# quanpn90/avsr

Hardware: AMD Instinct MI355X
Metric: AV-frames/sec/GPU (fwd+bwd) on 15s clips; WER parity on LRS2 test (higher is better)
Workload: dtype bf16

## Files before the change

### avsr_amd/csrc/gemm.hip

```cpp
#include "gemm_core.h"
#include "gemm_glds.h"
#include "gemm_pp.h"
#include <algorithm>
#include <cstring>

using namespace gemmcore;

namespace {

struct DenseArgs {
  int M, N, K, splits, kchunk;
  uint32_t a_bytes, b_bytes;
  int64_t sSplit;
  const void* A; int64_t lda, sA;
  const void* B; int64_t ldb, sB;
  int64_t sC, sR;
  Epi e;
  unsigned long long* stamp;
  unsigned* cnt;
  float* fC; int64_t fldc;
  float falpha, fbeta;
  const float* ln_c1; float ln_eps;
  float* lnst;
  float* kvk; float* kvv; const int* kvpos; int kvrows;
};

template <typename T, typename OutT, int WM, int WN, bool AK, bool BK>
__global__ __launch_bounds__(NT) void dense_kernel(DenseArgs a) {
  extern __shared__ __attribute__((aligned(16))) char smem[];
  using TL = Tile<T, WM, WN, AK, BK>;
  const int z = blockIdx.z, bz = z / a.splits, sp = z % a.splits;
  const int m0 = blockIdx.y * TL::BM, n0 = blockIdx.x * TL::BN;
  using LA = typename std::conditional<AK, LdDenseK<T, TL::BM>, LdDenseR<T, TL::BM>>::type;
  using LB = typename std::conditional<BK, LdDenseK<T, TL::BN>, LdDenseR<T, TL::BN>>::type;
  LA la; la.p = (const T*)a.A + (int64_t)bz * a.sA; la.ld = a.lda; la.rext = a.M; la.K = a.K;
  LB lb; lb.p = (const T*)a.B + (int64_t)bz * a.sB; lb.ld = a.ldb; lb.rext = a.N; lb.K = a.K;
  const int kbeg = sp * a.kchunk, kend = min(a.K, kbeg + a.kchunk);
  f32x16 acc[2][2];
  mainloop<T, WM, WN>(la, lb, m0, n0, kbeg, kend, acc, smem);
  Epi e = a.e;
  e.C = (OutT*)e.C + (int64_t)bz * a.sC + sp * a.sSplit;
  if (e.res) e.res = (const T*)e.res + (int64_t)bz * a.sR;
  if (e.preact) e.preact = (T*)e.preact + (int64_t)bz * a.sC;
  if (e.gate) e.gate = (const T*)e.gate + (int64_t)bz * a.sC;
  e.drop_base = (uint64_t)bz * (uint64_t)a.M * (uint64_t)a.N;
  epilogue<T, OutT, WM, WN>(e, m0, n0, acc, smem);
}

template <typename OutT, bool AK, bool BK, class CF>
__global__ __launch_bounds__(CF::NTH, CF::MINB) void dense_glds_kernel(DenseArgs a, int tiles_m, int tiles_n) {
  extern __shared__ __attribute__((aligned(16))) char smem[];
  if (a.stamp != nullptr && threadIdx.x == 0) atomicMin(a.stamp, (unsigned long long)__builtin_amdgcn_s_memrealtime());
  const int id = gemmg::xcd_remap(blockIdx.x, gridDim.x);
  int tm, tn, z;
  gemmg::tile_of(id, tiles_m, tiles_n, tm, tn, z);
  const int bz = z / a.splits, sp = z % a.splits;
  const int m0 = tm * CF::BM, n0 = tn * CF::BN;
  const int kbeg = sp * a.kchunk, kend = min(a.K, kbeg + a.kchunk);
  const int lane = threadIdx.x & 63, wave = __builtin_amdgcn_readfirstlane(threadIdx.x >> 6);
  f32x4 acc[CF::TM][CF::TN];
  const int nk = (kend - kbeg + gemmg::GBK - 1) / gemmg::GBK;
  if (a.a_bytes) {
    using LA = typename std::conditional<AK, gemmg::BDenseK<CF::BM, CF::NW>, gemmg::BDenseR<CF::BM, CF::NW>>::type;
    using LB = typename std::conditional<BK, gemmg::BDenseK<CF::BN, CF::NW>, gemmg::BDenseR<CF::BN, CF::NW>>::type;
    LA la; la.init((const bf16*)a.A + (int64_t)bz * a.sA, a.a_bytes, a.lda, m0, a.M, kend, wave, lane);
    LB lb; lb.init((const bf16*)a.B + (int64_t)bz * a.sB, a.b_bytes, a.ldb, n0, a.N, kend, wave, lane);
    gemmg::mainloop_glds<CF>(la, lb, kbeg, nk, acc, smem);
  } else {
    using LA = typename std::conditional<AK, gemmg::GDenseK<CF::BM, CF::NW>, gemmg::GDenseR<CF::BM, CF::NW>>::type;
    using LB = typename std::conditional<BK, gemmg::GDenseK<CF::BN, CF::NW>, gemmg::GDenseR<CF::BN, CF::NW>>::type;
    LA la; la.init((const bf16*)a.A + (int64_t)bz * a.sA, a.lda, m0, a.M, kend, wave, lane);
    LB lb; lb.init((const bf16*)a.B + (int64_t)bz * a.sB, a.ldb, n0, a.N, kend, wave, lane);
    gemmg::mainloop_glds<CF>(la, lb, kbeg, nk, acc, smem);
  }
  Epi e = a.e;
  e.C = (OutT*)e.C + (int64_t)bz * a.sC + sp * a.sSplit;
  if (e.res) e.res = (const bf16*)e.res + (int64_t)bz * a.sR;
  if (e.preact) e.preact = (bf16*)e.preact + (int64_t)bz * a.sC;
  if (e.gate) e.gate = (const bf16*)e.gate + (int64_t)bz * a.sC;
  e.drop_base = (uint64_t)bz * (uint64_t)a.M * (uint64_t)a.N;
  gemmg::epilogue_g<bf16, OutT, CF>(e, m0, n0, acc, smem);
  if (a.stamp != nullptr) {
    __syncthreads();
    if (threadIdx.x == 0) atomicMax(a.stamp + 1, (unsigned long long)__builtin_amdgcn_s_memrealtime());
  }
}

template <class CF, bool FR>
__device__ __forceinline__ void wgrad_dual_body(const DenseArgs& a, int tiles_m, int tiles_n, int id, char* smem) {
  static_assert(CF::BM * (CF::BN + 4) * 4 <= 2 * CF::S * CF::STAGE, "reduction tile exceeds the two rings");
  if (a.stamp != nullptr && threadIdx.x == 0) atomicMin(a.stamp, (unsigned long long)__builtin_amdgcn_s_memrealtime());
  int tm, tn, sp;
  if (a.cnt) {
    int z;
    gemmg::tile_of(id / a.splits, tiles_m, tiles_n, tm, tn, z);
    sp = id % a.splits;
  } else {
    gemmg::tile_of(id, tiles_m, tiles_n, tm, tn, sp);
  }
  const int m0 = tm * CF::BM, n0 = tn * CF::BN;
  const int kbeg = sp * a.kchunk, kend = min(a.K, kbeg + a.kchunk);
  const int lane = threadIdx.x & 63;
  const int wv = __builtin_amdgcn_readfirstlane(threadIdx.x >> 6);
  const int grp = wv >> 2, wave = wv & 3;
  const int ntile = (kend - kbeg + gemmg::GBK - 1) / gemmg::GBK;
  const int nk = (ntile + 1) >> 1;
  const int gbeg = kbeg + grp * nk * gemmg::GBK, gend = min(kend, gbeg + nk * gemmg::GBK);
  f32x4 acc[CF::TM][CF::TN];
  char* ring = smem + grp * (CF::S * CF::STAGE);
  if (a.a_bytes) {
    gemmg::BDenseR<CF::BM, CF::NW> la; la.init((const bf16*)a.A, a.a_bytes, a.lda, m0, a.M, gend, wave, lane);
    gemmg::BDenseR<CF::BN, CF::NW> lb; lb.init((const bf16*)a.B, a.b_bytes, a.ldb, n0, a.N, gend, wave, lane);
    gemmg::mainloop_glds<CF>(la, lb, gbeg, nk, acc, ring, wave);
  } else {
    gemmg::GDenseR<CF::BM, CF::NW> la; la.init((const bf16*)a.A, a.lda, m0, a.M, gend, wave, lane);
    gemmg::GDenseR<CF::BN, CF::NW> lb; lb.init((const bf16*)a.B, a.ldb, n0, a.N, gend, wave, lane);
    gemmg::mainloop_glds<CF>(la, lb, gbeg, nk, acc, ring, wave);
  }
  constexpr int LDR = CF::BN + 4;
  float* st = (float*)smem;
  const int wm = wave / CF::WN, wn = wave % CF::WN;
#pragma unroll
  for (int i = 0; i < CF::TM; ++i)
#pragma unroll
    for (int j = 0; j < CF::TN; ++j)
#pragma unroll
      for (int r = 0; r < 4; ++r) {
        const int row = wm * 32 * CF::FM + 16 * i + 4 * (lane >> 4) + r, col = wn * 32 * CF::FN + 16 * j + (lane & 15);
        if (grp == 0) st[row * LDR + col] = acc[i][j][r];
      }
  __syncthreads();
#pragma unroll
  for (int i = 0; i < CF::TM; ++i)
#pragma unroll
    for (int j = 0; j < CF::TN; ++j)
#pragma unroll
      for (int r = 0; r < 4; ++r) {
        const int row = wm * 32 * CF::FM + 16 * i + 4 * (lane >> 4) + r, col = wn * 32 * CF::FN + 16 * j + (lane & 15);
        if (grp == 1) st[row * LDR + col] += acc[i][j][r];
      }
  __syncthreads();
  const bool slab = a.sSplit != 0;
  constexpr int Q = CF::BN / 4;
  if constexpr (FR) {
    float* W = (float*)a.e.C;
    const int64_t ldw = a.e.ldc;
    const __amdgpu_buffer_rsrc_t rs = gemmg::make_rsrc(W, (uint32_t)((int64_t)a.splits * a.sSplit * 4));
    for (int c = threadIdx.x; c < CF::BM * Q; c += 2 * CF::NTH) {
      const int lr = c / Q, lc = (c % Q) * 4, row = m0 + lr, col = n0 + lc;
      if (row >= a.M || col >= a.N) continue;
      const f32x4 v = *(const f32x4*)(st + lr * LDR + lc);
      const uint32_t off = (uint32_t)((sp * a.sSplit + (int64_t)row * ldw + col) * 4);
      __builtin_amdgcn_raw_buffer_store_b128(__builtin_bit_cast(v4i32, v), rs, off, 0, 16 );
    }
    asm volatile("s_waitcnt vmcnt(0)" ::: "memory");
    __shared__ int last;
    __syncthreads();
    const int tile = tm * tiles_n + tn;
    if (threadIdx.x == 0)
      last = __hip_atomic_fetch_add(&a.cnt[tile], 1u, __ATOMIC_RELAXED, __HIP_MEMORY_SCOPE_AGENT) == (unsigned)a.splits - 1;
    __syncthreads();
    if (last) {
      constexpr int NI = CF::BM * Q / (2 * CF::NTH), SMAX = 4;
      static_assert(NI * 2 * CF::NTH == CF::BM * Q, "tile vectors per thread");
// ... 54 lines not shown
    }
    return;
  }
  float* C = slab ? (float*)a.e.C + sp * a.sSplit : (float*)a.e.C;
  const int64_t ldc = a.e.ldc;
  const float alpha = slab ? 1.f : a.e.alpha, beta = slab ? 0.f : a.e.beta;
  for (int c = threadIdx.x; c < CF::BM * Q; c += 2 * CF::NTH) {
    const int lr = c / Q, lc = (c % Q) * 4, row = m0 + lr, col = n0 + lc;
    if (row >= a.M || col >= a.N) continue;
    const f32x4 v = *(const f32x4*)(st + lr * LDR + lc);
    float* o = C + (int64_t)row * ldc + col;
    if (col + 4 <= a.N) {
      f32x4 y = v * alpha;
      if (beta != 0.f) y += *(const f32x4*)o * beta;
      *(f32x4*)o = y;
    } else {
      for (int q = 0; q < a.N - col; ++q) o[q] = beta != 0.f ? alpha * v[q] + beta * o[q] : alpha * v[q];
    }
  }
  if (a.stamp != nullptr) {
    __syncthreads();
    if (threadIdx.x == 0) atomicMax(a.stamp + 1, (unsigned long long)__builtin_amdgcn_s_memrealtime());
  }
}

template <class CF, bool FR = false>
__global__ __launch_bounds__(2 * CF::NTH, 1) void wgrad_dual_kernel(DenseArgs a, int tiles_m, int tiles_n) {
  extern __shared__ __attribute__((aligned(16))) char smem[];
  wgrad_dual_body<CF, FR>(a, tiles_m, tiles_n, gemmg::xcd_remap(blockIdx.x, gridDim.x), smem);
}

constexpr int WG_MAX = 4;
struct WgGroup {
  DenseArgs a[WG_MAX];
  int tm[WG_MAX], tn[WG_MAX], start[WG_MAX + 1];
};
template <class CF>
__global__ __launch_bounds__(2 * CF::NTH, 1) void wgrad_group_kernel(WgGroup g) {
  extern __shared__ __attribute__((aligned(16))) char smem[];
  const int id = gemmg::xcd_remap(blockIdx.x, gridDim.x);
  int q = 0;
#pragma unroll
  for (int i = 1; i < WG_MAX; ++i) q += id >= g.start[i];
  q = __builtin_amdgcn_readfirstlane(q);
  wgrad_dual_body<CF, false>(g.a[q], g.tm[q], g.tn[q], id - g.start[q], smem);
}

template <typename OutT, bool AK, bool BK>
__global__ __launch_bounds__(gemmpp::NTH, 1) void dense_pp_kernel(DenseArgs a, int tiles_m, int tiles_n) {
  extern __shared__ __attribute__((aligned(16))) char smem[];
  const int id = gemmg::xcd_remap(blockIdx.x, gridDim.x);
  int tm, tn, z;
  gemmg::tile_of(id, tiles_m, tiles_n, tm, tn, z);
  const int bz = z / a.splits, sp = z % a.splits;
  const int m0 = tm * gemmpp::BM, n0 = tn * gemmpp::BN;
  const int kbeg = sp * a.kchunk, kend = min(a.K, kbeg + a.kchunk);
  const int lane = threadIdx.x & 63, wave = __builtin_amdgcn_readfirstlane(threadIdx.x >> 6);
  using LA = typename std::conditional<AK, gemmpp::HalfK<64>, gemmpp::HalfR<64>>::type;
  using LB = typename std::conditional<BK, gemmpp::HalfK<32>, gemmpp::HalfR<32>>::type;
  LA la; la.init((const bf16*)a.A + (int64_t)bz * a.sA, a.lda, m0, a.M, kend, wave, lane);
  LB lb; lb.init((const bf16*)a.B + (int64_t)bz * a.sB, a.ldb, n0, a.N, kend, wave, lane);
  f32x4 acc[8][4];
  gemmpp::mainloop_pp(la, lb, kbeg, (kend - kbeg + gemmg::GBK - 1) / gemmg::GBK, acc, smem);
  Epi e = a.e;
  e.C = (OutT*)e.C + (int64_t)bz * a.sC + sp * a.sSplit;
  if (e.res) e.res = (const bf16*)e.res + (int64_t)bz * a.sR;
  if (e.preact) e.preact = (bf16*)e.preact + (int64_t)bz * a.sC;
  if (e.gate) e.gate = (const bf16*)e.gate + (int64_t)bz * a.sC;
  e.drop_base = (uint64_t)bz * (uint64_t)a.M * (uint64_t)a.N;
  gemmg::epilogue_g<bf16, OutT, gemmpp::CF>(e, m0, n0, acc, smem);
}

template <typename OutT, bool AK, bool BK>
int launch_pp(const DenseArgs& a, int batch, hipStream_t st) {
  const int tm = (a.M + 255) / 256, tn = (a.N + 255) / 256;
  const long nwg = (long)tm * tn * batch * a.splits;
  if (nwg > 0x7fffffffL) return AVSR_E_SHAPE;
  hipLaunchKernelGGL((dense_pp_kernel<OutT, AK, BK>), dim3((unsigned)nwg), dim3(gemmpp::NTH), gemmpp::LDS_BYTES, st, a,
                     tm, tn);
  AVSR_CHECK_LAUNCH();
  return 0;
}

template <typename OutT, bool AK, bool BK, class CF>
int launch_glds(const DenseArgs& a, int batch, hipStream_t st) {
  const int tm = (a.M + CF::BM - 1) / CF::BM, tn = (a.N + CF::BN - 1) / CF::BN;
  const long nwg = (long)tm * tn * batch * a.splits;
  if (nwg > 0x7fffffffL) return AVSR_E_SHAPE;
  hipLaunchKernelGGL((dense_glds_kernel<OutT, AK, BK, CF>), dim3((unsigned)nwg), dim3(CF::NTH), CF::LDS_BYTES, st, a,
                     tm, tn);
  AVSR_CHECK_LAUNCH();
  return 0;
}

using Cfg128 = gemmg::GCfg<2, 2, 2, 2, 2>;
using Cfg256 = gemmg::GCfg<2, 4, 4, 2, 2>;
using Cfg256x128 = gemmg::GCfg<4, 2, 2, 2, 3>;
using Cfg128x256 = gemmg::GCfg<2, 4, 2, 2, 3>;
using Cfg128s3 = gemmg::GCfg<2, 2, 2, 2, 3>;
using Cfg128s4 = gemmg::GCfg<2, 2, 2, 2, 4>;
using Cfg128w8s3 = gemmg::GCfg<2, 4, 2, 1, 3>;
using Cfg128w8s4 = gemmg::GCfg<2, 4, 2, 1, 4>;
using Cfg96 = gemmg::GCfg<3, 2, 1, 2, 2>;
using Cfg128x64 = gemmg::GCfg<4, 1, 1, 2, 2>;
using Cfg192 = gemmg::GCfg<2, 2, 3, 2, 2>;
using Cfg192x256 = gemmg::GCfg<2, 4, 3, 2, 2>;
using Cfg192s3 = gemmg::GCfg<2, 2, 3, 2, 3>;
using Cfg192w8 = gemmg::GCfg<2, 4, 3, 1, 2>;
using Cfg192w8s3 = gemmg::GCfg<2, 4, 3, 1, 3>;
using Cfg64 = gemmg::GCfg<2, 2, 1, 1, 2>;
using Cfg64s4 = gemmg::GCfg<2, 2, 1, 1, 4>;
using Cfg192w8s4 = gemmg::GCfg<2, 4, 3, 1, 4>;

#ifndef AVSR_AB_FWD2
#define AVSR_AB_FWD2 11
#endif
#ifndef AVSR_AB_ROUND1
#define AVSR_AB_ROUND1 15
#endif
int tile_cfg(const avsr_gemm_params* p, int splits) {
  const int forced = (int)avsr_opt(AVSR_OPT_GEMM_TILE) - 1;
  if (forced >= 0) return forced;
  if (p->a_kmajor) {
    const long tiles_z = (long)p->batch * splits;
    const long t128 = (long)((p->M + 127) / 128) * ((p->N + 127) / 128) * tiles_z;
    const long t192 = (long)((p->M + 191) / 192) * ((p->N + 127) / 128) * tiles_z;
    const long n128 = (t128 + 255) / 256, n192 = (t192 + 255) / 256;
    if (n192 >= 2 && 3 * n192 * 50 <= 2 * n128 * 51) return AVSR_AB_FWD2;
    if (t192 > 128 && t192 <= 256) return AVSR_AB_ROUND1;
  }
  {
    const long tiles_z = (long)p->batch * splits;
    const long t128 = (long)((p->M + 127) / 128) * ((p->N + 127) / 128) * tiles_z;
    const long t64 = (long)((p->M + 63) / 64) * ((p->N + 63) / 64) * tiles_z;
    if (t128 < 256 && t64 >= 2 * t128) return (t64 <= 256 && p->K >= 2048) ? 18 : 16;
  }
  return 0;
}

int cfg_bm(int cfg, bool ak) {
  switch (cfg) {
    case 1: return Cfg256::BM;
    case 2: return Cfg256x128::BM;
    case 3: return Cfg128x256::BM;
    case 4: return Cfg128s3::BM;
    case 5: return Cfg128s4::BM;
    case 6: return Cfg128w8s3::BM;
    case 7: return Cfg128w8s4::BM;
    case 8: return gemmpp::BM;
    case 9: return ak ? Cfg96::BM : Cfg128::BM;
    case 10: return Cfg128x64::BM;
    case 16: return Cfg64::BM;
    case 18: return Cfg64s4::BM;
    case 11: return ak ? Cfg192::BM : Cfg128::BM;
    case 12: return ak ? Cfg192x256::BM : Cfg128::BM;
    case 13: return ak ? Cfg192s3::BM : Cfg128::BM;
    case 14: return ak ? Cfg192w8::BM : Cfg128::BM;
    case 15: return ak ? Cfg192w8s3::BM : Cfg128::BM;
    case 17: return ak ? Cfg192w8s4::BM : Cfg128::BM;
    default: return Cfg128::BM;
  }
}

template <typename OutT, bool AK, bool BK>
int launch_cfg(int cfg, const DenseArgs& a, int batch, hipStream_t st) {
  switch (cfg) {
    case 1: return launch_glds<OutT, AK, BK, Cfg256>(a, batch, st);
    case 2: return launch_glds<OutT, AK, BK, Cfg256x128>(a, batch, st);
    case 3: return launch_glds<OutT, AK, BK, Cfg128x256>(a, batch, st);
    case 4: return launch_glds<OutT, AK, BK, Cfg128s3>(a, batch, st);
    case 5: return launch_glds<OutT, AK, BK, Cfg128s4>(a, batch, st);
    case 6: return launch_glds<OutT, AK, BK, Cfg128w8s3>(a, batch, st);
    case 7: return launch_glds<OutT, AK, BK, Cfg128w8s4>(a, batch, st);
    case 8: return launch_pp<OutT, AK, BK>(a, batch, st);
    case 9:
      if constexpr (AK) return launch_glds<OutT, AK, BK, Cfg96>(a, batch, st);
      else return launch_glds<OutT, AK, BK, Cfg128>(a, batch, st);
    case 10: return launch_glds<OutT, AK, BK, Cfg128x64>(a, batch, st);
    case 16: return launch_glds<OutT, AK, BK, Cfg64>(a, batch, st);
    case 18: return launch_glds<OutT, AK, BK, Cfg64s4>(a, batch, st);
    case 11:
      if constexpr (AK) return launch_glds<OutT, AK, BK, Cfg192>(a, batch, st);
      else return launch_glds<OutT, AK, BK, Cfg128>(a, batch, st);
    case 12:
      if constexpr (AK) return launch_glds<OutT, AK, BK, Cfg192x256>(a, batch, st);
      else return launch_glds<OutT, AK, BK, Cfg128>(a, batch, st);
    case 13:
      if constexpr (AK) return launch_glds<OutT, AK, BK, Cfg192s3>(a, batch, st);
      else return launch_glds<OutT, AK, BK, Cfg128>(a, batch, st);
    case 14:
      if constexpr (AK) return launch_glds<OutT, AK, BK, Cfg192w8>(a, batch, st);
      else return launch_glds<OutT, AK, BK, Cfg128>(a, batch, st);
    case 15:
      if constexpr (AK) return launch_glds<OutT, AK, BK, Cfg192w8s3>(a, batch, st);
      else return launch_glds<OutT, AK, BK, Cfg128>(a, batch, st);
    case 17:
      if constexpr (AK) return launch_glds<OutT, AK, BK, Cfg192w8s4>(a, batch, st);
      else return launch_glds<OutT, AK, BK, Cfg128>(a, batch, st);
    default: return launch_glds<OutT, AK, BK, Cfg128>(a, batch, st);
  }
}

template <typename OutT>
int glds_by_layout(const avsr_gemm_params* p, const DenseArgs& a, hipStream_t st) {
  const int cfg = tile_cfg(p, a.splits);
  if (p->a_kmajor && p->b_kmajor) return launch_cfg<OutT, true, true>(cfg, a, p->batch, st);
  if (p->a_kmajor) return launch_cfg<OutT, true, false>(cfg, a, p->batch, st);
  if (p->b_kmajor) return launch_cfg<OutT, false, true>(cfg, a, p->batch, st);
  return launch_cfg<OutT, false, false>(cfg, a, p->batch, st);
}

bool glds_ok(const avsr_gemm_params* p) {
  if (p->dtype != AVSR_BF16 || p->M < 128 || p->N < 128) return false;
  if (!p->a_kmajor && (p->M % 8)) return false;
  if (!p->b_kmajor && (p->N % 8)) return false;
  return true;
}

template <typename T, typename OutT, int WM, int WN, bool AK, bool BK>
int launch(const DenseArgs& a, int batch, hipStream_t st) {
  using TL = Tile<T, WM, WN, AK, BK>;
  dim3 grid((a.N + TL::BN - 1) / TL::BN, (a.M + TL::BM - 1) / TL::BM, batch * a.splits);
  hipLaunchKernelGGL((dense_kernel<T, OutT, WM, WN, AK, BK>), grid, dim3(NT), TL::LDS_BYTES, st, a);
  AVSR_CHECK_LAUNCH();
  return 0;
}

template <typename T, typename OutT, int WM, int WN>
int by_layout(const avsr_gemm_params* p, const DenseArgs& a, hipStream_t st) {
  if (p->a_kmajor && p->b_kmajor) return launch<T, OutT, WM, WN, true, true>(a, p->batch, st);
  if (p->a_kmajor) return launch<T, OutT, WM, WN, true, false>(a, p->batch, st);
  if (p->b_kmajor) return launch<T, OutT, WM, WN, false, true>(a, p->batch, st);
  return launch<T, OutT, WM, WN, false, false>(a, p->batch, st);
}

template <typename T, typename OutT>
int by_tile(const avsr_gemm_params* p, const DenseArgs& a, hipStream_t st) {
  if (p->N <= 64) return by_layout<T, OutT, 4, 1>(p, a, st);
  if (p->M <= 64) return by_layout<T, OutT, 1, 4>(p, a, st);
  return by_layout<T, OutT, 2, 2>(p, a, st);
}

constexpr int SK_NB = 16;

template <typename T> AVSR_DEV f32x4 ld4f(const T* p) {
  if constexpr (sizeof(T) == 2) {
    const bf16x4 v = *(const bf16x4*)p;
    return f32x4{(float)v[0], (float)v[1], (float)v[2], (float)v[3]};
  } else {
    return *(const f32x4*)p;
  }
}

template <typename T, typename OutT, int MR>
__global__ __launch_bounds__(256) void skinny_kernel(DenseArgs a, float* part, int kchunk, unsigned* cnt) {
  constexpr int SK_KC = MR <= 32 ? 256 : 128;
  constexpr int XPT = MR * SK_KC / 4 / 256;
  constexpr int WJ = SK_KC / 128;
  __shared__ __attribute__((aligned(16))) float xs[MR][SK_KC + 4];
  static_assert(4 * MR * (SK_NB + 1) <= MR * (SK_KC + 4), "reduction slab reuses the staging buffer");
  float (*red)[MR][SK_NB + 1] = (float (*)[MR][SK_NB + 1])&xs[0][0];
  const int tid = threadIdx.x, cg = tid & 7, kl = tid >> 3, lane = tid & 63, wave = tid >> 6;
  const int n0 = blockIdx.x * SK_NB, c0 = n0 + 2 * cg, c1 = c0 + 1;
  const T* A = (const T*)a.A;
  const T* B0 = (const T*)a.B + (int64_t)min(c0, a.N - 1) * a.ldb;
  const T* B1 = (const T*)a.B + (int64_t)min(c1, a.N - 1) * a.ldb;
  const bool ok0 = c0 < a.N, ok1 = c1 < a.N;
  float acc0[MR], acc1[MR];
#pragma unroll
  for (int m = 0; m < MR; ++m) acc0[m] = acc1[m] = 0.f;
  const int kbeg = part ? blockIdx.y * kchunk : 0;
  const int kend = part ? min(a.K, kbeg + kchunk) : a.K;
  f32x4 xr[XPT], w0[WJ], w1[WJ];
  auto load = [&](int k0) {
#pragma unroll
    for (int i = 0; i < XPT; ++i) {
      const int idx = tid + 256 * i, m = idx / (SK_KC / 4), q = idx - m * (SK_KC / 4), k = k0 + 4 * q;
// ... 551 lines not shown
```

### avsr_amd/csrc/gemm_core.h

```cpp
#pragma once
#include "common.h"

namespace gemmcore {

constexpr int BKE = 32, NT = 256;

template <typename T> struct V { static constexpr int VE = 16 / (int)sizeof(T); static constexpr int ROW = BKE + VE; };

AVSR_DEV void zero(v16& v) { v.w[0] = v.w[1] = v.w[2] = v.w[3] = 0u; }

struct ConvGeom {
  int nimg, hin, win, hout, wout;
  int kh, kw, sh, sw, ph, pw;
  int cin, cout;
  int64_t ldx, ldy;
  FastDiv f_hw_out, f_w_out;
  FastDiv f_hw_in, f_w_in;
  FastDiv f_kw;
  int cin_shift, cout_shift;
  int ktot_w, tap_kfw, tap_kh0, tap_kw0, tap_step;
};

template <typename T, int R> struct LdDenseK {
  static constexpr bool KMAJ = true;
// ... 251 lines not shown
  void* preact;
  const void* res; int64_t ldr;
  const void* gate;
  float drop_p; uint64_t seed; uint64_t drop_base;
  float* stats;
  int stats_tiles;
  int rm_wc, rm_hc, rm_hin, rm_win, rm_a, rm_b;
  float* colsum;
};

AVSR_DEV int epi_row(const Epi& e, int r) {
  if (e.rm_wc == 0) return r;
  const int q = r / e.rm_wc, j = r - q * e.rm_wc;
  const int n = q / e.rm_hc, i = q - n * e.rm_hc;
  return (n * e.rm_hin + 2 * i + e.rm_a) * e.rm_win + 2 * j + e.rm_b;
}

AVSR_DEV int acc_row(int wm, int i, int r, int lane) { return wm * 64 + i * 32 + (r & 3) + 8 * (r >> 2) + 4 * (lane >> 5); }
AVSR_DEV int acc_col(int wn, int j, int lane) { return wn * 64 + j * 32 + (lane & 31); }

template <typename T, typename OutT, int NE>
AVSR_DEV void epi_elems(const Epi& e, int row, int col, const float* v_in) {
  OutT* C = (OutT*)e.C;
  const T* R = (const T*)e.res;
  T* P = (T*)e.preact;
  const T* G = (const T*)e.gate;
  const int64_t off = (int64_t)row * e.ldc + col;
  if (e.atomic) {
#pragma unroll
    for (int q = 0; q < NE; ++q)
      if (col + q < e.N) atomicAdd((float*)C + off + q, e.alpha * v_in[q]);
    return;
  }
#pragma unroll
  for (int q = 0; q < NE; ++q) {
    if (col + q >= e.N) break;
    float v = e.alpha * v_in[q];
    const uint64_t didx = e.drop_base + (uint64_t)row * (uint64_t)e.N + col + q;
    if (!e.bwd) {
      if (e.bias) v += e.bias[col + q];
      if (P) P[off + q] = from_f<T>(v);
      v = act_fwd_t<T>(e.act, v);
      if (e.drop_p > 0.f) v *= drop_scale(e.drop_p, e.seed, didx);
      if (R) v += to_f(R[(int64_t)row * e.ldr + col + q]);
    } else {
      if (e.drop_p > 0.f) v *= drop_scale(e.drop_p, e.seed, didx);
      if (G) v *= act_bwd_t<T>(e.act, to_f(G[off + q]));
    }
    if (e.beta != 0.f) v += e.beta * to_f(C[off + q]);
    C[off + q] = from_f<OutT>(v);
  }
}

template <typename T, typename OutT>
AVSR_DEV bool epi_vec_ok(const Epi& e) {
  const uintptr_t a = (uintptr_t)e.C | (uintptr_t)e.preact | (uintptr_t)e.res | (uintptr_t)e.gate | (uintptr_t)e.bias;
  return !e.atomic && (a & 15u) == 0 && ((e.ldc * (int64_t)sizeof(OutT)) & 15) == 0 &&
         ((e.ldc * (int64_t)sizeof(T)) & 15) == 0 && ((e.ldr * (int64_t)sizeof(T)) & 15) == 0;
}

template <typename T> AVSR_DEV void ld8(const T* p, float (&o)[8]) {
  if constexpr (sizeof(T) == 2) {
    const bf16x8 x = *(const bf16x8*)p;
#pragma unroll
    for (int j = 0; j < 8; ++j) o[j] = (float)x[j];
  } else {
    const f32x4 x0 = *(const f32x4*)p, x1 = *(const f32x4*)(p + 4);
#pragma unroll
    for (int j = 0; j < 4; ++j) { o[j] = x0[j]; o[j + 4] = x1[j]; }
  }
}
template <typename T> AVSR_DEV void st8(T* p, const float (&o)[8]) {
  if constexpr (sizeof(T) == 2) {
    bf16x8 x;
#pragma unroll
    for (int j = 0; j < 8; ++j) x[j] = (bf16)o[j];
    *(bf16x8*)p = x;
  } else {
    *(f32x4*)p = f32x4{o[0], o[1], o[2], o[3]};
    *(f32x4*)(p + 4) = f32x4{o[4], o[5], o[6], o[7]};
  }
}

template <typename T, typename OutT>
AVSR_DEV void epi_vec8(const Epi& e, int row, int col, float (&v)[8]) {
  const int64_t off = (int64_t)row * e.ldc + col;
#pragma unroll
  for (int q = 0; q < 8; ++q) v[q] *= e.alpha;
  float t[8];
  const uint64_t d0 = e.drop_base + (uint64_t)row * (uint64_t)e.N + col;
  if (!e.bwd) {
    if (e.bias) {
      ld8(e.bias + col, t);
#pragma unroll
      for (int q = 0; q < 8; ++q) v[q] += t[q];
    }
    if (e.preact) st8((T*)e.preact + off, v);
    if (e.act) {
      if (sizeof(T) == 2 && e.act == AVSR_ACT_GELU) {
#pragma unroll
        for (int q = 0; q < 8; q += 2) {
          const f32x2 r = gelu_fast2(f32x2{v[q], v[q + 1]});
          v[q] = r.x; v[q + 1] = r.y;
        }
      } else {
#pragma unroll
        for (int q = 0; q < 8; ++q) v[q] = act_fwd_t<T>(e.act, v[q]);
      }
    }
    if (e.drop_p > 0.f) drop8(e.drop_p, e.seed, d0, v);
    if (e.res) {
      ld8((const T*)e.res + (int64_t)row * e.ldr + col, t);
#pragma unroll
      for (int q = 0; q < 8; ++q) v[q] += t[q];
    }
  } else {
    if (e.drop_p > 0.f) drop8(e.drop_p, e.seed, d0, v);
    if (e.gate) {
      ld8((const T*)e.gate + off, t);
      if (sizeof(T) == 2 && e.act == AVSR_ACT_GELU) {
#pragma unroll
        for (int q = 0; q < 8; q += 2) {
          const f32x2 r = gelu_fast_grad2(f32x2{t[q], t[q + 1]});
          v[q] *= r.x; v[q + 1] *= r.y;
        }
      } else {
#pragma unroll
        for (int q = 0; q < 8; ++q) v[q] *= act_bwd_t<T>(e.act, t[q]);
      }
    }
  }
  if (e.beta != 0.f) {
    ld8((const OutT*)e.C + off, t);
#pragma unroll
    for (int q = 0; q < 8; ++q) v[q] += e.beta * t[q];
  }
  st8((OutT*)e.C + off, v);
}

template <typename T, typename OutT, int WM, int WN>
AVSR_DEV void epilogue(const Epi& e, int m0, int n0, f32x16 (&acc)[2][2], char* smem) {
  constexpr int BM = 64 * WM, BN = 64 * WN, HR = BM / 2, LDR = BN + 4;
  const int tid = threadIdx.x, lane = tid & 63, wid = tid >> 6;
  const int wm = wid / WN, wn = wid % WN;
  float* st = (float*)smem;
  if (e.stats) {
    __syncthreads();
    float* red = st;
#pragma unroll
    for (int j = 0; j < 2; ++j) {
      float s = 0.f, c = 0.f;
#pragma unroll
      for (int i = 0; i < 2; ++i)
#pragma unroll
        for (int r = 0; r < 16; ++r) {
          const bool ok = m0 + acc_row(wm, i, r, lane) < e.M;
          s += ok ? e.alpha * acc[i][j][r] : 0.f;
          c += ok ? 1.f : 0.f;
        }
      s += __shfl_xor(s, 32, 64);
      c += __shfl_xor(c, 32, 64);
      const float mean = c > 0.f ? s / c : 0.f;
      float m2 = 0.f;
#pragma unroll
      for (int i = 0; i < 2; ++i)
#pragma unroll
        for (int r = 0; r < 16; ++r) {
          const bool ok = m0 + acc_row(wm, i, r, lane) < e.M;
          const float d = e.alpha * acc[i][j][r] - mean;
          m2 += ok ? d * d : 0.f;
        }
      m2 += __shfl_xor(m2, 32, 64);
      if (lane < 32) {
        const int lc = acc_col(wn, j, lane);
        red[(wm * BN + lc) * 3 + 0] = c;
        red[(wm * BN + lc) * 3 + 1] = mean;
        red[(wm * BN + lc) * 3 + 2] = m2;
      }
    }
    __syncthreads();
    for (int lc = tid; lc < BN; lc += NT) {
      const int col = n0 + lc;
      if (col < e.N) {
        float n = 0.f, mean = 0.f, m2 = 0.f;
        for (int w = 0; w < WM; ++w) {
          const float nb = red[(w * BN + lc) * 3 + 0], mb = red[(w * BN + lc) * 3 + 1], qb = red[(w * BN + lc) * 3 + 2];
          if (nb > 0.f) {
            const float nn = n + nb, d = mb - mean;
            mean += d * nb / nn;
            m2 += qb + d * d * n * nb / nn;
            n = nn;
          }
        }
        float* o = e.stats + ((int64_t)col * e.stats_tiles + m0 / BM) * 3;
        o[0] = n; o[1] = mean; o[2] = m2;
      }
    }
  }
#pragma unroll
  for (int half = 0; half < 2; ++half) {
    __syncthreads();
#pragma unroll
// ... 40 lines not shown
```

### avsr_amd/csrc/gemm_glds.h

```cpp
#pragma once
#include "gemm_core.h"

namespace gemmg {
using namespace gemmcore;

constexpr int GBK = 64;

static __device__ __attribute__((aligned(16))) uint4 g_zero_line[64];

typedef __attribute__((address_space(3))) void lds_void_t;
typedef const __attribute__((address_space(1))) void gbl_void_t;

AVSR_DEV void glds16(const void* src, char* lds_wave_base) {
  __builtin_amdgcn_global_load_lds((gbl_void_t*)src, (lds_void_t*)lds_wave_base, 16, 0, 0);
}

template <int CPR> AVSR_DEV int rswz(int k) {
  return CPR >= 16 ? ((k & 3) | (((k >> 3) & 1) << 2)) << 1 : (((k >> 1) & 1) | (((k >> 3) & 1) << 1)) << 1;
}

template <int R, int NW> struct GDenseK {
  static constexpr bool KMAJ = true;
  static constexpr int SLOTS = R / 8 / NW;
  const bf16* p[SLOTS];
// ... 142 lines not shown
  static constexpr int LDS_BYTES = S * STAGE > EP_BYTES ? S * STAGE : EP_BYTES;
  static constexpr int MINB = LDS_BYTES <= 53 * 1024 ? 3 : LDS_BYTES <= 80 * 1024 ? 2 : 1;
  static constexpr int TM = 2 * FM, TN = 2 * FN;
};

template <int N> AVSR_DEV void wait_vmcnt() { asm volatile("s_waitcnt vmcnt(%0)" ::"n"(N) : "memory"); }

template <class CF, bool AK, bool BK>
struct Frags {
  bf16x8 a[CF::TM], b[CF::TN];
  AVSR_DEV void load(const char* stage, int kb, int wm, int wn, int lane) {
#pragma unroll
    for (int i = 0; i < CF::TM; ++i) a[i] = gfrag<CF::BM, AK>(stage, (wm * CF::TM + i) * 16, kb, lane);
#pragma unroll
    for (int j = 0; j < CF::TN; ++j) b[j] = gfrag<CF::BN, BK>(stage + CF::SA, (wn * CF::TN + j) * 16, kb, lane);
  }
  AVSR_DEV void mma(f32x4 (&acc)[CF::TM][CF::TN]) const {
#pragma unroll
    for (int i = 0; i < CF::TM; ++i)
#pragma unroll
      for (int j = 0; j < CF::TN; ++j) acc[i][j] = mfma16(a[i], b[j], acc[i][j]);
  }
};

template <class CF>
AVSR_DEV void wait_tiles_ahead(bool full) {
  if (full) wait_vmcnt<CF::GL * (CF::S - 2)>();
  else wait_vmcnt<0>();
}

template <class CF, class LA, class LB>
AVSR_DEV void mainloop_glds(const LA& la, const LB& lb, int kbeg, int nk, f32x4 (&acc)[CF::TM][CF::TN], char* smem,
                            int wave) {
  constexpr int S = CF::S, KS = GBK / 32;
  const int lane = threadIdx.x & 63;
  const int wm = wave / CF::WN, wn = wave % CF::WN;
#pragma unroll
  for (int i = 0; i < CF::TM; ++i)
#pragma unroll
    for (int j = 0; j < CF::TN; ++j) acc[i][j] = f32x4{0.f, 0.f, 0.f, 0.f};
  if (nk <= 0) return;
#pragma unroll
  for (int p = 0; p < S; ++p)
    if (p < nk) {
      la.issue(smem + p * CF::STAGE, kbeg + p * GBK, wave);
      lb.issue(smem + p * CF::STAGE + CF::SA, kbeg + p * GBK, wave);
    }
  if (nk >= S) wait_vmcnt<CF::GL * (S - 1)>();
  else wait_vmcnt<0>();
  __builtin_amdgcn_s_barrier();
  asm volatile("" ::: "memory");
  static_assert(KS == 2, "the fragment sets alternate over two k-steps per K-tile");
  Frags<CF, LA::KMAJ, LB::KMAJ> f0, f1;
  f0.load(smem, 0, wm, wn, lane);
  int cs = 0;
  for (int kt = 0; kt < nk; ++kt) {
    const char* stage = smem + cs * CF::STAGE;
    const int ns = cs + 1 == S ? 0 : cs + 1;
    f1.load(stage, 1, wm, wn, lane);
    f0.mma(acc);
    if (kt + 1 < nk) {
      asm volatile("s_waitcnt lgkmcnt(0)" ::: "memory");
      wait_tiles_ahead<CF>(kt + S - 1 < nk);
      __builtin_amdgcn_s_barrier();
      asm volatile("" ::: "memory");
      if (kt + S < nk) {
        char* st = smem + cs * CF::STAGE;
        la.issue(st, kbeg + (kt + S) * GBK, wave);
        lb.issue(st + CF::SA, kbeg + (kt + S) * GBK, wave);
      }
      f0.load(smem + ns * CF::STAGE, 0, wm, wn, lane);
    }
    f1.mma(acc);
    cs = ns;
  }
  __syncthreads();
}

template <class CF, class LA, class LB>
AVSR_DEV void mainloop_glds(const LA& la, const LB& lb, int kbeg, int nk, f32x4 (&acc)[CF::TM][CF::TN], char* smem) {
  mainloop_glds<CF>(la, lb, kbeg, nk, acc, smem, __builtin_amdgcn_readfirstlane(threadIdx.x >> 6));
}

template <typename T, typename OutT, class CF>
AVSR_DEV void epilogue_g(const Epi& e, int m0, int n0, f32x4 (&acc)[CF::TM][CF::TN], char* smem) {
  constexpr int BN = CF::BN, LDR = BN + 4, SR = CF::WM * 32;
  const int tid = threadIdx.x, lane = tid & 63, wave = tid >> 6;
  const int wm = wave / CF::WN, wn = wave % CF::WN;
  float* st = (float*)smem;
  const bool vec = epi_vec_ok<T, OutT>(e);
  if (e.stats) {
    __syncthreads();
    float* red = st;
#pragma unroll
    for (int j = 0; j < CF::TN; ++j) {
      float s = 0.f, c = 0.f;
#pragma unroll
      for (int i = 0; i < CF::TM; ++i)
#pragma unroll
        for (int r = 0; r < 4; ++r) {
          const int row = wm * 32 * CF::FM + i * 16 + 4 * (lane >> 4) + r;
          const bool ok = m0 + row < e.M;
          s += ok ? e.alpha * acc[i][j][r] : 0.f;
          c += ok ? 1.f : 0.f;
        }
      s += __shfl_xor(s, 16, 64); s += __shfl_xor(s, 32, 64);
      c += __shfl_xor(c, 16, 64); c += __shfl_xor(c, 32, 64);
      const float mean = c > 0.f ? s / c : 0.f;
      float m2 = 0.f;
#pragma unroll
      for (int i = 0; i < CF::TM; ++i)
#pragma unroll
        for (int r = 0; r < 4; ++r) {
          const int row = wm * 32 * CF::FM + i * 16 + 4 * (lane >> 4) + r;
          const float d = e.alpha * acc[i][j][r] - mean;
          m2 += m0 + row < e.M ? d * d : 0.f;
        }
      m2 += __shfl_xor(m2, 16, 64); m2 += __shfl_xor(m2, 32, 64);
      if (lane < 16) {
        const int lc = (wn * CF::TN + j) * 16 + lane;
        red[(wm * BN + lc) * 3 + 0] = c;
        red[(wm * BN + lc) * 3 + 1] = mean;
        red[(wm * BN + lc) * 3 + 2] = m2;
      }
    }
    __syncthreads();
    for (int lc = tid; lc < BN; lc += CF::NTH) {
      const int col = n0 + lc;
      if (col < e.N) {
        float n = 0.f, mean = 0.f, m2 = 0.f;
        for (int w = 0; w < CF::WM; ++w) {
          const float nb = red[(w * BN + lc) * 3 + 0], mb = red[(w * BN + lc) * 3 + 1], qb = red[(w * BN + lc) * 3 + 2];
          if (nb > 0.f) {
            const float nn = n + nb, d = mb - mean;
            mean += d * nb / nn;
            m2 += qb + d * d * n * nb / nn;
            n = nn;
          }
        }
        float* o = e.stats + ((int64_t)col * e.stats_tiles + m0 / CF::BM) * 3;
        o[0] = n; o[1] = mean; o[2] = m2;
      }
    }
  }
  static_assert(CF::NTH % (BN / 8) == 0, "a thread's column group must be fixed");
  float cs[8];
#pragma unroll
  for (int j = 0; j < 8; ++j) cs[j] = 0.f;
#pragma unroll
  for (int i = 0; i < CF::FM; ++i) {
    __syncthreads();
#pragma unroll
    for (int h = 0; h < 2; ++h)
#pragma unroll
      for (int j = 0; j < CF::TN; ++j)
#pragma unroll
        for (int r = 0; r < 4; ++r) {
          const int lr = wm * 32 + h * 16 + 4 * (lane >> 4) + r;
          st[lr * LDR + (wn * CF::TN + j) * 16 + (lane & 15)] = acc[2 * i + h][j][r];
        }
    __syncthreads();
    for (int c = tid; c < SR * BN / 8; c += CF::NTH) {
      const int lr = c / (BN / 8), lc = (c % (BN / 8)) * 8;
      const int row = m0 + ((lr >> 5) * CF::FM + i) * 32 + (lr & 31);
      const int col = n0 + lc;
      if (row < e.M && col < e.N) {
        const f32x4 v0 = *(const f32x4*)(st + lr * LDR + lc), v1 = *(const f32x4*)(st + lr * LDR + lc + 4);
        float v[8] = {v0[0], v0[1], v0[2], v0[3], v1[0], v1[1], v1[2], v1[3]};
        const int orow = epi_row(e, row);
        if (vec && col + 8 <= e.N) {
          epi_vec8<T, OutT>(e, orow, col, v);
          if (e.colsum) {
#pragma unroll
            for (int j = 0; j < 8; ++j) cs[j] += v[j];
          }
        } else {
          epi_elems<T, OutT, 4>(e, orow, col, v);
          if (col + 4 < e.N) epi_elems<T, OutT, 4>(e, orow, col + 4, v + 4);
        }
      }
    }
  }
  if (e.colsum) {
    constexpr int CG = BN / 8, RP = 9;
    __syncthreads();
#pragma unroll
    for (int j = 0; j < 8; ++j) st[tid * RP + j] = cs[j];
    __syncthreads();
    for (int t = tid; t < BN; t += CF::NTH) {
      const int g = t >> 3, j = t & 7;
      float s = 0.f;
      for (int k = g; k < CF::NTH; k += CG) s += st[k * RP + j];
      if (n0 + t < e.N) e.colsum[(int64_t)(m0 / CF::BM) * e.N + n0 + t] = s;
    }
  }
}

struct BnrArgs {
  const bf16* h; const bf16* res;
  const float *scale, *shift, *prelu, *mean, *invstd, *scale2, *shift2, *mean2, *invstd2;
  float* ws;
};

template <class CF, int RES>
AVSR_DEV void epilogue_bnr(const Epi& e, const BnrArgs& b, int m0, int n0, f32x4 (&acc)[CF::TM][CF::TN], char* smem) {
  constexpr int BN = CF::BN, LDR = BN + 4, SR = CF::WM * 32, CG = BN / 8, RP = 33, IT = SR * CG / CF::NTH;
  static_assert(CF::NTH % CG == 0 && (SR * CG) % CF::NTH == 0, "a thread's column group must be fixed");
  static_assert(CF::NTH * RP * 4 <= CF::LDS_BYTES, "partials staging exceeds LDS");
  const int tid = threadIdx.x, lane = tid & 63, wave = tid >> 6;
  const int wm = wave / CF::WN, wn = wave % CF::WN;
  float* st = (float*)smem;
  const int lc = (tid % CG) * 8, col = n0 + lc;
  const bool colok = col < e.N;
  const bool beta = e.beta != 0.f, alpha1 = e.alpha == 1.f;
  float sc[8], sh[8], pw[8], mu[8], is[8], sc2[8], sh2[8], mu2[8], is2[8];
#pragma unroll
  for (int j = 0; j < 8; ++j) {
    const int c = colok ? col + j : 0;
    sc[j] = b.scale[c]; sh[j] = b.shift[c]; pw[j] = b.prelu[c]; mu[j] = b.mean[c]; is[j] = b.invstd[c];
    if constexpr (RES == 2) { sc2[j] = b.scale2[c]; sh2[j] = b.shift2[c]; mu2[j] = b.mean2[c]; is2[j] = b.invstd2[c]; }
  }
  float s0[8], s1[8], s2[8], s3[8];
#pragma unroll
  for (int j = 0; j < 8; ++j) s0[j] = s1[j] = s2[j] = s3[j] = 0.f;
  bf16* C = (bf16*)e.C;
#pragma unroll
  for (int i = 0; i < CF::FM; ++i) {
    bf16x8 ph[IT], pr[IT], pc[IT];
    int64_t off[IT];
    bool ok[IT];
#pragma unroll
    for (int it = 0; it < IT; ++it) {
      const int lr = (tid + it * CF::NTH) / CG;
      const int row = m0 + ((lr >> 5) * CF::FM + i) * 32 + (lr & 31);
      ok[it] = row < e.M && colok;
      off[it] = ok[it] ? (int64_t)epi_row(e, row) * e.ldc + col : 0;
      ph[it] = *(const bf16x8*)(b.h + off[it]);
      if constexpr (RES != 0) pr[it] = *(const bf16x8*)(b.res + off[it]);
      if (beta) pc[it] = *(const bf16x8*)(C + off[it]);
    }
    __syncthreads();
#pragma unroll
    for (int h = 0; h < 2; ++h)
#pragma unroll
// ... 81 lines not shown
```

Measured before the change: 141,900.

## Specialize GEMM epilogue per fused-op variant with hoisted bias and prefetched operands

Adds compile-time epilogue variants (plain, bias, bias+residual, bias+GELU with preact, backward GELU gate), selected on the host from the epilogue flags and pointer alignment, for two dense GEMM tile configs. Each specialized kernel drops runtime branches and generic paths. It loads the bias vector once per thread and prefetches residual or gate rows before the LDS staging barrier, so those global loads overlap the accumulator spill. The cost is more kernel instantiations, extra registers for the prefetched data, and a host-side dispatch that has to match the device fold exactly.

New measurement: 145,000 (median of 6 runs). 2.2% higher.

```diff
diff --git a/avsr_amd/csrc/gemm.hip b/avsr_amd/csrc/gemm.hip
--- a/avsr_amd/csrc/gemm.hip
+++ b/avsr_amd/csrc/gemm.hip
@@ -47,7 +47,19 @@
   epilogue<T, OutT, WM, WN>(e, m0, n0, acc, smem);
 }
 
-template <typename OutT, bool AK, bool BK, class CF>
+template <typename OutT, int EV>
+AVSR_DEV Epi tile_epi(const DenseArgs& a, int bz, int sp) {
+  Epi e = a.e;
+  epi_fold<EV>(e);
+  e.C = (OutT*)e.C + (int64_t)bz * a.sC + sp * a.sSplit;
+  if (e.res) e.res = (const bf16*)e.res + (int64_t)bz * a.sR;
+  if (e.preact) e.preact = (bf16*)e.preact + (int64_t)bz * a.sC;
+  if (e.gate) e.gate = (const bf16*)e.gate + (int64_t)bz * a.sC;
+  e.drop_base = (uint64_t)bz * (uint64_t)a.M * (uint64_t)a.N;
+  return e;
+}
+
+template <typename OutT, bool AK, bool BK, class CF, int EV = EV_GENERIC>
 __global__ __launch_bounds__(CF::NTH, CF::MINB) void dense_glds_kernel(DenseArgs a, int tiles_m, int tiles_n) {
   extern __shared__ __attribute__((aligned(16))) char smem[];
   if (a.stamp != nullptr && threadIdx.x == 0) atomicMin(a.stamp, (unsigned long long)__builtin_amdgcn_s_memrealtime());
@@ -73,13 +85,8 @@
     LB lb; lb.init((const bf16*)a.B + (int64_t)bz * a.sB, a.ldb, n0, a.N, kend, wave, lane);
     gemmg::mainloop_glds<CF>(la, lb, kbeg, nk, acc, smem);
   }
-  Epi e = a.e;
-  e.C = (OutT*)e.C + (int64_t)bz * a.sC + sp * a.sSplit;
-  if (e.res) e.res = (const bf16*)e.res + (int64_t)bz * a.sR;
-  if (e.preact) e.preact = (bf16*)e.preact + (int64_t)bz * a.sC;
-  if (e.gate) e.gate = (const bf16*)e.gate + (int64_t)bz * a.sC;
-  e.drop_base = (uint64_t)bz * (uint64_t)a.M * (uint64_t)a.N;
-  gemmg::epilogue_g<bf16, OutT, CF>(e, m0, n0, acc, smem);
+  const Epi e = tile_epi<OutT, EV>(a, bz, sp);
+  gemmg::epilogue_g<bf16, OutT, CF, EV>(e, m0, n0, acc, smem);
   if (a.stamp != nullptr) {
     __syncthreads();
     if (threadIdx.x == 0) atomicMax(a.stamp + 1, (unsigned long long)__builtin_amdgcn_s_memrealtime());
@@ -300,11 +307,65 @@
   return 0;
 }
 
-template <typename OutT, bool AK, bool BK, class CF>
+template <typename OutT>
+int epi_variant(const DenseArgs& a, int batch) {
+  const Epi& e = a.e;
+  if (e.atomic || e.stats || e.rm_wc || e.alpha != 1.f || e.beta != 0.f || (e.N % 8)) return EV_GENERIC;
+  const uintptr_t ptrs = (uintptr_t)e.C | (uintptr_t)e.preact | (uintptr_t)e.res | (uintptr_t)e.gate | (uintptr_t)e.bias;
+  if (ptrs & 15u) return EV_GENERIC;
+  const int64_t so = (int64_t)sizeof(OutT);
+  if (((e.ldc * so) | (e.ldc * 2) | (e.ldr * 2)) & 15) return EV_GENERIC;
+  if (batch > 1 && (((a.sC * so) | (a.sC * 2) | (a.sR * 2)) & 15)) return EV_GENERIC;
+  if (a.splits > 1 && ((a.sSplit * so) & 15)) return EV_GENERIC;
+  const bool drop = e.drop_p > 0.f;
+  if (!e.bwd) {
+    if (e.gate || e.colsum) return EV_GENERIC;
+    if (!e.bias) return (!e.preact && !e.act && !e.res && !drop) ? EV_PLAIN : EV_GENERIC;
+    if (!e.preact && !e.act && !e.res && !drop) return EV_BIAS;
+    if (!e.preact && !e.act && e.res) return EV_BIAS_RES;
+    if (e.preact && e.act == AVSR_ACT_GELU && !e.res) return EV_BIAS_ACT_PRE;
+    return EV_GENERIC;
+  }
+  if (e.bias || e.preact || e.res) return EV_GENERIC;
+  if (e.gate && e.act == AVSR_ACT_GELU) return EV_GATE;
+  if (!e.gate && !e.act && !drop && !e.colsum) return EV_PLAIN;
+  return EV_GENERIC;
+}
+
+template <typename OutT, bool BK, int EV>
+constexpr bool ev_built() {
+  if (EV == EV_GENERIC) return true;
+  if (sizeof(OutT) != 2) return false;
+  return BK ? (EV == EV_BIAS || EV == EV_BIAS_RES || EV == EV_BIAS_ACT_PRE) : (EV == EV_PLAIN || EV == EV_GATE);
+}
+
+template <typename OutT, bool AK, bool BK, class CF, int EV>
+int launch_glds_ev(const DenseArgs& a, int tm, int tn, long nwg, hipStream_t st) {
+  if constexpr (!ev_built<OutT, BK, EV>()) {
+    return launch_glds_ev<OutT, AK, BK, CF, EV_GENERIC>(a, tm, tn, nwg, st);
+  } else {
+    hipLaunchKernelGGL((dense_glds_kernel<OutT, AK, BK, CF, EV>), dim3((unsigned)nwg), dim3(CF::NTH), CF::LDS_BYTES,
+                       st, a, tm, tn);
+    AVSR_CHECK_LAUNCH();
+    return 0;
+  }
+}
+
+template <typename OutT, bool AK, bool BK, class CF, bool VARIANTS = false>
 int launch_glds(const DenseArgs& a, int batch, hipStream_t st) {
   const int tm = (a.M + CF::BM - 1) / CF::BM, tn = (a.N + CF::BN - 1) / CF::BN;
   const long nwg = (long)tm * tn * batch * a.splits;
   if (nwg > 0x7fffffffL) return AVSR_E_SHAPE;
+  if constexpr (VARIANTS) {
+    switch (epi_variant<OutT>(a, batch)) {
+      case EV_PLAIN: return launch_glds_ev<OutT, AK, BK, CF, EV_PLAIN>(a, tm, tn, nwg, st);
+      case EV_BIAS: return launch_glds_ev<OutT, AK, BK, CF, EV_BIAS>(a, tm, tn, nwg, st);
+      case EV_BIAS_RES: return launch_glds_ev<OutT, AK, BK, CF, EV_BIAS_RES>(a, tm, tn, nwg, st);
+      case EV_BIAS_ACT_PRE: return launch_glds_ev<OutT, AK, BK, CF, EV_BIAS_ACT_PRE>(a, tm, tn, nwg, st);
+      case EV_GATE: return launch_glds_ev<OutT, AK, BK, CF, EV_GATE>(a, tm, tn, nwg, st);
+      default: break;
+    }
+  }
   hipLaunchKernelGGL((dense_glds_kernel<OutT, AK, BK, CF>), dim3((unsigned)nwg), dim3(CF::NTH), CF::LDS_BYTES, st, a,
                      tm, tn);
   AVSR_CHECK_LAUNCH();
@@ -398,7 +459,7 @@
     case 16: return launch_glds<OutT, AK, BK, Cfg64>(a, batch, st);
     case 18: return launch_glds<OutT, AK, BK, Cfg64s4>(a, batch, st);
     case 11:
-      if constexpr (AK) return launch_glds<OutT, AK, BK, Cfg192>(a, batch, st);
+      if constexpr (AK) return launch_glds<OutT, AK, BK, Cfg192, true>(a, batch, st);
       else return launch_glds<OutT, AK, BK, Cfg128>(a, batch, st);
     case 12:
       if constexpr (AK) return launch_glds<OutT, AK, BK, Cfg192x256>(a, batch, st);
@@ -410,7 +471,7 @@
       if constexpr (AK) return launch_glds<OutT, AK, BK, Cfg192w8>(a, batch, st);
       else return launch_glds<OutT, AK, BK, Cfg128>(a, batch, st);
     case 15:
-      if constexpr (AK) return launch_glds<OutT, AK, BK, Cfg192w8s3>(a, batch, st);
+      if constexpr (AK) return launch_glds<OutT, AK, BK, Cfg192w8s3, true>(a, batch, st);
       else return launch_glds<OutT, AK, BK, Cfg128>(a, batch, st);
     case 17:
       if constexpr (AK) return launch_glds<OutT, AK, BK, Cfg192w8s4>(a, batch, st);
diff --git a/avsr_amd/csrc/gemm_core.h b/avsr_amd/csrc/gemm_core.h
--- a/avsr_amd/csrc/gemm_core.h
+++ b/avsr_amd/csrc/gemm_core.h
@@ -357,8 +357,29 @@
   }
 }
 
+enum { EV_GENERIC = 0, EV_PLAIN = 1, EV_BIAS = 2, EV_BIAS_RES = 3, EV_BIAS_ACT_PRE = 4, EV_GATE = 5 };
+
+template <int EV> AVSR_DEV void epi_fold(Epi& e) {
+  if constexpr (EV != EV_GENERIC) {
+    e.alpha = 1.f; e.beta = 0.f; e.atomic = 0; e.stats = nullptr; e.rm_wc = 0;
+    e.bwd = EV == EV_GATE;
+    if constexpr (EV == EV_PLAIN || EV == EV_GATE) e.bias = nullptr;
+    else __builtin_assume(e.bias != nullptr);
+    if constexpr (EV == EV_BIAS_ACT_PRE) __builtin_assume(e.preact != nullptr);
+    else e.preact = nullptr;
+    if constexpr (EV == EV_BIAS_RES) __builtin_assume(e.res != nullptr);
+    else e.res = nullptr;
+    if constexpr (EV == EV_GATE) __builtin_assume(e.gate != nullptr);
+    else e.gate = nullptr;
+    e.act = (EV == EV_BIAS_ACT_PRE || EV == EV_GATE) ? AVSR_ACT_GELU : AVSR_ACT_NONE;
+    if constexpr (EV == EV_PLAIN || EV == EV_BIAS) e.drop_p = 0.f;
+    if constexpr (EV != EV_GATE) e.colsum = nullptr;
+  }
+}
+
 template <typename T, typename OutT>
-AVSR_DEV void epi_vec8(const Epi& e, int row, int col, float (&v)[8]) {
+AVSR_DEV void epi_vec8(const Epi& e, int row, int col, float (&v)[8], const float* bv = nullptr,
+                       const bf16x8* op = nullptr) {
   const int64_t off = (int64_t)row * e.ldc + col;
 #pragma unroll
   for (int q = 0; q < 8; ++q) v[q] *= e.alpha;
@@ -366,7 +387,12 @@
   const uint64_t d0 = e.drop_base + (uint64_t)row * (uint64_t)e.N + col;
   if (!e.bwd) {
     if (e.bias) {
-      ld8(e.bias + col, t);
+      if (bv) {
+#pragma unroll
+        for (int q = 0; q < 8; ++q) t[q] = bv[q];
+      } else {
+        ld8(e.bias + col, t);
+      }
 #pragma unroll
       for (int q = 0; q < 8; ++q) v[q] += t[q];
     }
@@ -385,14 +411,24 @@
     }
     if (e.drop_p > 0.f) drop8(e.drop_p, e.seed, d0, v);
     if (e.res) {
-      ld8((const T*)e.res + (int64_t)row * e.ldr + col, t);
+      if (op) {
+#pragma unroll
+        for (int q = 0; q < 8; ++q) t[q] = (float)(*op)[q];
+      } else {
+        ld8((const T*)e.res + (int64_t)row * e.ldr + col, t);
+      }
 #pragma unroll
       for (int q = 0; q < 8; ++q) v[q] += t[q];
     }
   } else {
     if (e.drop_p > 0.f) drop8(e.drop_p, e.seed, d0, v);
     if (e.gate) {
-      ld8((const T*)e.gate + off, t);
+      if (op) {
+#pragma unroll
+        for (int q = 0; q < 8; ++q) t[q] = (float)(*op)[q];
+      } else {
+        ld8((const T*)e.gate + off, t);
+      }
       if (sizeof(T) == 2 && e.act == AVSR_ACT_GELU) {
 #pragma unroll
         for (int q = 0; q < 8; q += 2) {
diff --git a/avsr_amd/csrc/gemm_glds.h b/avsr_amd/csrc/gemm_glds.h
--- a/avsr_amd/csrc/gemm_glds.h
+++ b/avsr_amd/csrc/gemm_glds.h
@@ -248,13 +248,13 @@
   mainloop_glds<CF>(la, lb, kbeg, nk, acc, smem, __builtin_amdgcn_readfirstlane(threadIdx.x >> 6));
 }
 
-template <typename T, typename OutT, class CF>
+template <typename T, typename OutT, class CF, int EV = EV_GENERIC>
 AVSR_DEV void epilogue_g(const Epi& e, int m0, int n0, f32x4 (&acc)[CF::TM][CF::TN], char* smem) {
   constexpr int BN = CF::BN, LDR = BN + 4, SR = CF::WM * 32;
   const int tid = threadIdx.x, lane = tid & 63, wave = tid >> 6;
   const int wm = wave / CF::WN, wn = wave % CF::WN;
   float* st = (float*)smem;
-  const bool vec = epi_vec_ok<T, OutT>(e);
+  const bool vec = EV != EV_GENERIC || epi_vec_ok<T, OutT>(e);
   if (e.stats) {
     __syncthreads();
     float* red = st;
@@ -313,8 +313,30 @@
   float cs[8];
 #pragma unroll
   for (int j = 0; j < 8; ++j) cs[j] = 0.f;
+  constexpr int CGV = BN / 8, IT = SR * CGV / CF::NTH;
+  constexpr bool PREB = EV == EV_BIAS || EV == EV_BIAS_RES || EV == EV_BIAS_ACT_PRE;
+  constexpr bool PREOP = (EV == EV_BIAS_RES || EV == EV_GATE) && sizeof(T) == 2;
+  static_assert(EV == EV_GENERIC || IT * CF::NTH == SR * CGV, "whole vectors per thread per strip");
+  const int lc0 = (tid % CGV) * 8;
+  float bv[8];
+  if constexpr (PREB) {
+    if (n0 + lc0 < e.N) ld8(e.bias + n0 + lc0, bv);
+  }
 #pragma unroll
   for (int i = 0; i < CF::FM; ++i) {
+    bf16x8 pre[PREOP ? IT : 1];
+    if constexpr (PREOP) {
+#pragma unroll
+      for (int it = 0; it < IT; ++it) {
+        const int lr = (tid + it * CF::NTH) / CGV;
+        const int row = m0 + ((lr >> 5) * CF::FM + i) * 32 + (lr & 31);
+        if (row < e.M && n0 + lc0 < e.N) {
+          const int orow = epi_row(e, row);
+          pre[it] = EV == EV_GATE ? *(const bf16x8*)((const bf16*)e.gate + (int64_t)orow * e.ldc + n0 + lc0)
+                                  : *(const bf16x8*)((const bf16*)e.res + (int64_t)orow * e.ldr + n0 + lc0);
+        }
+      }
+    }
     __syncthreads();
 #pragma unroll
     for (int h = 0; h < 2; ++h)
@@ -326,6 +348,23 @@
           st[lr * LDR + (wn * CF::TN + j) * 16 + (lane & 15)] = acc[2 * i + h][j][r];
         }
     __syncthreads();
+    if constexpr (EV != EV_GENERIC) {
+#pragma unroll
+      for (int it = 0; it < IT; ++it) {
+        const int lr = (tid + it * CF::NTH) / CGV;
+        const int row = m0 + ((lr >> 5) * CF::FM + i) * 32 + (lr & 31);
+        const int col = n0 + lc0;
+        if (row < e.M && col < e.N) {
+          const f32x4 v0 = *(const f32x4*)(st + lr * LDR + lc0), v1 = *(const f32x4*)(st + lr * LDR + lc0 + 4);
+          float v[8] = {v0[0], v0[1], v0[2], v0[3], v1[0], v1[1], v1[2], v1[3]};
+          epi_vec8<T, OutT>(e, epi_row(e, row), col, v, PREB ? bv : nullptr, PREOP ? &pre[it] : nullptr);
+          if (e.colsum) {
+#pragma unroll
+            for (int j = 0; j < 8; ++j) cs[j] += v[j];
+          }
+        }
+      }
+    } else
     for (int c = tid; c < SR * BN / 8; c += CF::NTH) {
       const int lr = c / (BN / 8), lc = (c % (BN / 8)) * 8;
       const int row = m0 + ((lr >> 5) * CF::FM + i) * 32 + (lr & 31);
```
